# sjtuytc/betapose

Measured on AMD Instinct MI355X. Metric: frames/sec (640x480, 50-kp KPD), higher is better.
Workload: dtype f32 as an exact 3-way bf16 operand split (6 bf16 MFMA products), f32 accumulate and activations

## Files before the change

betapose_amd/_lib.py:

```python
from __future__ import annotations

import ctypes as C
import os
import threading

_HERE = os.path.dirname(os.path.abspath(__file__))
LIB_PATH = os.environ.get("BP_LIB") or os.path.join(_HERE, "libbetapose_hip.so")
_lock = threading.Lock()
_lib = None

c_float_p = C.POINTER(C.c_float)
c_double_p = C.POINTER(C.c_double)
c_int_p = C.POINTER(C.c_int)
vp = C.c_void_p

PROTOTYPES = {
    "bp_last_error": (C.c_char_p, []),
    "bp_version": (C.c_int, []),
    "bp_device_count": (C.c_int, []),
    "bp_device_name": (C.c_int, [C.c_int, C.c_char_p, C.c_int]),
    "bp_yolo_create": (C.c_int, [C.c_char_p, C.c_char_p, C.c_int, C.c_int, C.c_int, C.POINTER(vp)]),
    "bp_yolo_create_from_memory": (C.c_int, [C.c_char_p, vp, C.c_size_t, C.c_int, C.c_int, C.c_int, C.POINTER(vp)]),
    "bp_yolo_clone": (C.c_int, [vp, C.POINTER(vp)]),
    "bp_kpd_clone": (C.c_int, [vp, C.POINTER(vp)]),
    "bp_yolo_destroy": (None, [vp]),
    "bp_yolo_rows": (C.c_int, [vp]),
    "bp_yolo_attrs": (C.c_int, [vp]),
    "bp_yolo_forward": (C.c_int, [vp, vp, C.c_int, vp, vp]),
    "bp_yolo_forward_select": (C.c_int, [vp, vp, C.c_int, C.c_float, C.c_int, vp, vp, vp]),
    "bp_yolo_forward_select_classes": (C.c_int, [vp, vp, C.c_int, C.c_float, C.c_int, vp, C.c_int, vp, vp, vp]),
    "bp_yolo_select": (C.c_int, [vp, C.c_int, C.c_int, C.c_int, C.c_float, C.c_int, vp, vp]),
    "bp_yolo_tap_count": (C.c_int, [vp]),
    "bp_yolo_tap_info": (C.c_int, [vp, C.c_int, C.c_char_p, C.c_int, c_int_p, c_int_p, c_int_p]),
    "bp_yolo_tap_copy": (C.c_int, [vp, C.c_int, C.c_int, vp, vp]),
    "bp_kpd_create": (C.c_int, [vp, C.c_size_t, C.c_int, C.c_int, C.c_int, C.POINTER(vp)]),
    "bp_kpd_destroy": (None, [vp]),
    "bp_kpd_forward": (C.c_int, [vp, vp, C.c_int, vp, vp]),
    "bp_kpd_forward_argmax": (C.c_int, [vp, vp, C.c_int, vp, vp, vp]),
    "bp_kpd_launch_count": (C.c_int, [vp, C.c_int]),
    "bp_kpd_tap_count": (C.c_int, [vp]),
    "bp_kpd_tap_info": (C.c_int, [vp, C.c_int, C.c_char_p, C.c_int, c_int_p, c_int_p, c_int_p]),
    "bp_kpd_tap_copy": (C.c_int, [vp, C.c_int, C.c_int, vp, vp]),
    "bp_yolo_set_policy": (C.c_int, [vp, C.c_int, C.c_int, C.c_int, C.c_int]),
    "bp_kpd_set_policy": (C.c_int, [vp, C.c_int, C.c_int, C.c_int, C.c_int]),
    "bp_yolo_set_precision": (C.c_int, [vp, C.c_int]),
    "bp_kpd_set_precision": (C.c_int, [vp, C.c_int]),
# ... 204 lines not shown
```

betapose_amd/csrc/aux_kernels.hip:

```cpp
#include "bp_common.h"

namespace bp {

__device__ __forceinline__ void store_plane(unsigned short* planes, long long idx, long long plane_elems, int np, float v) {
    if (np == 1) {
        const _Float16 h = (_Float16)v;
        planes[idx] = __builtin_bit_cast(unsigned short, h);
    } else if (np == 3) {
        const __bf16 h1 = (__bf16)v;
        const float r1 = v - (float)h1;
        const __bf16 h2 = (__bf16)r1;
        const __bf16 h3 = (__bf16)(r1 - (float)h2);
        planes[idx] = __builtin_bit_cast(unsigned short, h1);
        planes[idx + plane_elems] = __builtin_bit_cast(unsigned short, h2);
        planes[idx + 2 * plane_elems] = __builtin_bit_cast(unsigned short, h3);
    }
}

static inline int grid_for(long long n, int block = 256, int cap = 4096) {
    BP_CHECK(n < (1ll << 31), "tensor too large for 32-bit indexing");
    long long g = (n + block - 1) / block;
    return (int)(g < 1 ? 1 : (g > cap ? cap : g));
}

// ... 300 lines not shown
            o[1] = q[0] - q[2] / 2;
            o[2] = q[1] - q[3] / 2;
            o[3] = q[0] + q[2] / 2;
            o[4] = q[1] + q[3] / 2;
            o[5] = q[4];
            o[6] = q[5];
            o[7] = 0.f;
        }
    }
}
void launch_yolo_select(const float* pred, int N, int rows, int attrs, float conf, int num_classes, float* sel,
                        hipStream_t s, int sel_ld) {
    hipLaunchKernelGGL(yolo_select_kernel, dim3(N), dim3(1024), 0, s, pred, rows, attrs, conf, num_classes, sel, sel_ld);
}

__global__ __launch_bounds__(1024) void yolo_decode_select_kernel(YoloHeads hs, int reso, int attrs, int rows, float conf, int num_classes,
                                                                   float* __restrict__ sel, int sel_ld) {
    __shared__ float sv[16];
    __shared__ int si[16];
    const int n = blockIdx.x;
    const int ncls = min(num_classes, attrs - 5);
    auto locate = [&](int row, int* a) -> const float* {
        int hi = 0;
        for (int k = 1; k < hs.n; ++k)
            if (row >= hs.h[k].row_off) hi = k;
        const YoloHead& H = hs.h[hi];
        const int g = H.g, r = row - H.row_off;
        *a = r / (g * g);
        const int cell = r - *a * g * g;
        return H.t + ((long long)n * g * g + cell) * (3 * attrs) + *a * attrs;
    };
    float best = -1.f;
    int bi = 0x7fffffff;
    for (int r = threadIdx.x; r < rows; r += blockDim.x) {
        int a;
        const float* t = locate(r, &a);
        const float obj = sigmoidf_(t[4]);
        if (!(obj > conf)) continue;
        int cls = 0;
        float cm = sigmoidf_(t[5]);
        for (int k = 1; k < ncls; ++k) {
            const float v = sigmoidf_(t[5 + k]);
            if (v > cm) { cm = v; cls = k; }
        }
        if (cls != 0) continue;
        if (obj > best || (obj == best && r < bi)) { best = obj; bi = r; }
    }
    for (int off = 32; off > 0; off >>= 1) {
        const float ov = __shfl_down(best, off, 64);
        const int oi = __shfl_down(bi, off, 64);
        if (ov > best || (ov == best && oi < bi)) { best = ov; bi = oi; }
    }
    const int w = threadIdx.x >> 6;
    if ((threadIdx.x & 63) == 0) { sv[w] = best; si[w] = bi; }
    __syncthreads();
    if (threadIdx.x == 0) {
        for (int k = 1; k < (int)(blockDim.x >> 6); ++k)
            if (sv[k] > best || (sv[k] == best && si[k] < bi)) { best = sv[k]; bi = si[k]; }
        float* o = sel + (long long)n * sel_ld;
        if (best < 0.f) {
            o[0] = __int_as_float(-1);
            for (int k = 1; k < 8; ++k) o[k] = 0.f;
        } else {
            int a, hi = 0;
            const float* t = locate(bi, &a);
            for (int k = 1; k < hs.n; ++k)
                if (bi >= hs.h[k].row_off) hi = k;
            const YoloHead& H = hs.h[hi];
            const int g = H.g, r = bi - H.row_off, cell = r - a * g * g;
            const int gy = cell / g, gx = cell - gy * g;
            const float stride = (float)(reso / g);
            const float q0 = (sigmoidf_(t[0]) + (float)gx) * stride;
            const float q1 = (sigmoidf_(t[1]) + (float)gy) * stride;
            const float q2 = (expf(t[2]) * (H.aw[a] / stride)) * stride;
            const float q3 = (expf(t[3]) * (H.ah[a] / stride)) * stride;
            o[0] = __int_as_float(bi);
            o[1] = q0 - q2 / 2;
            o[2] = q1 - q3 / 2;
            o[3] = q0 + q2 / 2;
            o[4] = q1 + q3 / 2;
            o[5] = sigmoidf_(t[4]);
            o[6] = sigmoidf_(t[5]);
            o[7] = 0.f;
        }
    }
}
void launch_yolo_decode_select(const YoloHead* heads, int nheads, int N, int reso, int attrs, int rows, float conf, int num_classes,
                               float* sel, hipStream_t s, int sel_ld) {
    BP_CHECK(nheads <= 4, "at most 4 yolo heads");
    YoloHeads hs;
    hs.n = nheads;
    for (int i = 0; i < nheads; ++i) hs.h[i] = heads[i];
    hipLaunchKernelGGL(yolo_decode_select_kernel, dim3(N), dim3(1024), 0, s, hs, reso, attrs, rows, conf, num_classes, sel, sel_ld);
}

struct PredRows {
    const float* P;
    int attrs;
    __device__ __forceinline__ const float* row(int r) const { return P + (long long)r * attrs; }
    __device__ __forceinline__ float attr(const float* q, int k) const { return q[k]; }
    __device__ __forceinline__ void box(int, const float* q, float* b) const { b[0] = q[0]; b[1] = q[1]; b[2] = q[2]; b[3] = q[3]; }
};
struct HeadRows {
    const YoloHeads* hs;
    int n, attrs, reso;
    __device__ __forceinline__ int head_of(int r) const {
        int hi = 0;
        for (int k = 1; k < hs->n; ++k)
// ... 565 lines not shown
```

betapose_amd/csrc/bp_common.h:

```cpp
#pragma once
#include <hip/hip_runtime.h>
#include <cstdint>
#include <cstdio>
#include <mutex>
#include <set>
#include <stdexcept>
#include <string>
#include <utility>

namespace bp {

struct Error : std::runtime_error {
    using std::runtime_error::runtime_error;
};

#define BP_HIP(expr)                                                                      \
    do {                                                                                  \
        hipError_t _e = (expr);                                                           \
        if (_e != hipSuccess)                                                             \
            throw ::bp::Error(std::string(#expr) + ": " + hipGetErrorString(_e) + " @" +  \
                              __FILE__ + ":" + std::to_string(__LINE__));                 \
    } while (0)

#define BP_CHECK(cond, msg)                                                               \
// ... 61 lines not shown
    int out_np;
    int skip_f32;
    const unsigned short* res16;
    int net_prec;
    int abl;
    const unsigned short* wbd;
    const unsigned short* wpl;
    float* pool_out;
    int hy_full, hy_splits, hy_cps;
    int xcd_home;
    int* xcc_of;
    int* err_word;
    int* tickets_local;
    int mtiles, n_tiles;
    int work_blocks;
    const void* pf_ptr;
    int pf_first;
    int pf_ntn, pf_splits, pf_cps, pf_nchunks;
    int pf_tile_stride, pf_chunk_bytes;
    int pf_cap;
};

enum Precision : int { PREC_F32 = 0, PREC_F16 = 1, PREC_BF16X3 = 2, PREC_F16_RES = 3 };

enum ConvTile : int { TILE_64x64 = 0, TILE_128x64 = 1, TILE_W64_1x1 = 2, TILE_W64_1x2 = 3, TILE_W64_2x1 = 5, TILE_W64_2x2 = 6,
                      TILE_KG1 = 7, TILE_KG2 = 8, TILE_KG4 = 9,
                      TILE_RD4 = 10, TILE_RD8 = 11,
                      TILE_64x64_BD = 12,
                      TILE_PL64 = 13,
                      TILE_PL128 = 14,
// ... 87 lines not shown
int avgpool_parts(int HW);
void launch_avgpool(const float* in, int in_ld, float* out, int N, int HW, int C, hipStream_t s);
void launch_fc(const float* in, const float* w, const float* bias, float* out, int N, int Cin, int Cout,
               int act, int in_parts, float in_scale, hipStream_t s);

struct YoloHead {
    const float* t;
    int g;
    float aw[3], ah[3];
    int row_off;
};
void launch_yolo_decode(const YoloHead* heads, int nheads, int N, int reso, int attrs, int rows,
                        float* pred, hipStream_t s);
void launch_yolo_select(const float* pred, int N, int rows, int attrs, float conf, int num_classes,
                        float* sel, hipStream_t s, int sel_ld = 8);
void launch_yolo_decode_select(const YoloHead* heads, int nheads, int N, int reso, int attrs, int rows, float conf, int num_classes,
                               float* sel, hipStream_t s, int sel_ld = 8);
#define BP_MAX_SCENE_CLASSES 16
struct YoloClassList {
    int n;
    int id[BP_MAX_SCENE_CLASSES];
};
YoloClassList make_class_list(const int* class_ids, int K, int num_classes, int attrs);
void launch_yolo_select_classes(const float* pred, int N, int rows, int attrs, float conf, int num_classes, const YoloClassList& cl,
                                float* sel, hipStream_t s, int ld_image, int ld_slot);
void launch_yolo_decode_select_classes(const YoloHead* heads, int nheads, int N, int reso, int attrs, int rows, float conf,
                                       int num_classes, const YoloClassList& cl, float* sel, hipStream_t s, int ld_image, int ld_slot);
#define BP_MAX_CANDIDATES 8
void launch_yolo_select_nms(const float* pred, int N, int rows, int attrs, float conf, int num_classes, int class_id, float nms_conf,
                            int C, float* sel, int* count, hipStream_t s, int ld_image, int ld_slot);
void launch_yolo_decode_select_nms(const YoloHead* heads, int nheads, int N, int reso, int attrs, int rows, float conf, int num_classes,
                                   int class_id, float nms_conf, int C, float* sel, int* count, hipStream_t s, int ld_image,
// ... 27 lines not shown
```

betapose_amd/csrc/c_api.cpp:

```cpp
#include "../../include/betapose_hip.h"

#include <algorithm>
#include <cmath>
#include <cstdlib>
#include <cstring>
#include <fstream>
#include <memory>
#include <sstream>
#include <vector>

#include "annotate.h"
#include "engine.h"
#include "frame_chain.h"
#include "frame_io.h"
#include "icp.h"
#include "pose_tail.h"
#include "raster.h"

static thread_local std::string g_err;

#define BP_TRY try {
#define BP_CATCH                                   \
    }                                              \
    catch (const std::exception& e) {              \
// ... 333 lines not shown
                                   int K, float* d_pred, float* d_sel, void* stream) {
    BP_TRY
    BP_CHECK(K >= 1 && K <= BP_MAX_SCENE_CLASSES, "class list: 1 to 16 class ids (BP_MAX_SCENE_CLASSES)");
    BP_CHECK(y && d_img && class_ids && d_sel, "null argument");
    y->net->forward_classes(d_img, false, batch, d_pred, conf, num_classes, class_ids, K, d_sel, (hipStream_t)stream);
    return 0;
    BP_CATCH
}

int bp_yolo_select(const float* d_pred, int batch, int rows, int attrs, float conf, int num_classes, float* d_sel,
                   void* stream) {
    BP_TRY
    BP_CHECK(d_pred && d_sel && batch >= 1 && rows >= 1 && attrs >= 6, "bad argument");
    bp::launch_yolo_select(d_pred, batch, rows, attrs, conf, num_classes, d_sel, (hipStream_t)stream);
    BP_HIP(hipGetLastError());
    return 0;
    BP_CATCH
}

int bp_yolo_select_nms(const float* d_pred, int batch, int rows, int attrs, float conf, int num_classes, int class_id,
                       float nms_conf, int max_candidates, float* d_sel, int* d_counts, void* stream) {
    BP_TRY
    BP_CHECK(d_pred && d_sel && d_counts && batch >= 1 && rows >= 1 && attrs >= 6, "bad argument");
    bp::launch_yolo_select_nms(d_pred, batch, rows, attrs, conf, num_classes, class_id, nms_conf, max_candidates, d_sel, d_counts,
                               (hipStream_t)stream, max_candidates * BP_SEL_FLOATS, BP_SEL_FLOATS);
    BP_HIP(hipGetLastError());
    return 0;
    BP_CATCH
}

// ... 1529 lines not shown
```

betapose_amd/csrc/conv_igemm.hip:

```cpp
#include <cstdlib>

#include "conv_dev.h"

namespace bp {

template <int TM, int TN, int VEC, class P>
__device__ __forceinline__ void conv_igemm_body(const P& p, const int bp_bid, float* const smem, int* const s_last_p) {
    constexpr int BM = 64 * TM, BN = 64 * TN;
    constexpr int RA = BM / 32, RB = BN / 32;
    float (*As)[BM * LDS_LD] = reinterpret_cast<float (*)[BM * LDS_LD]>(smem);
    float (*Bs)[BN * LDS_LD] = reinterpret_cast<float (*)[BN * LDS_LD]>(smem + 2 * BM * LDS_LD);
    constexpr int LDT = BN + 4;
    static_assert(BM * LDT <= 2 * (BM + BN) * LDS_LD, "LDS too small for the staged epilogue");

    const unsigned long long t_entry = p.stamps ? bp_clock() : 0ull;
    const int tid = threadIdx.x;
    const int lane = tid & 63;
    const int wave = tid >> 6;
    const int wm = wave >> 1, wn = wave & 1;
    const int n_tiles_n = p.CoutPad / BN;
    const int split = bp_bid % p.splits;
    const int tile_id = bp_bid / p.splits;
    const int tile_n = tile_id % n_tiles_n;
    const int tile_m = tile_id / n_tiles_n;
// ... 488 lines not shown
        __syncthreads();
    }
#define BH_STAMP(k_) if (p.stamps && tid == 0) p.stamps[(long long)(tile_id * p.splits + split) * 8 + (k_)] = bp_clock();
    if (p.stamps && tid == 0) p.stamps[(long long)(tile_id * p.splits + split) * 8 + 0] = t_entry;
    BH_STAMP(3);

    const int w_row0 = wm * (BM / 2), w_col0 = wn * (BN / 2);
    const bool kg_has_acc = KG == 1 || kgrp == 0;
#define BP_NT (256 * KG)
#define BP_SLAST (*s_last_p)
#define BP_EARLY_BIAS bias_early
#define BP_HAS_ACC kg_has_acc
#define BP_TAIL_STAMP(k_) BH_STAMP(k_)
#define BP_EP_RES_SCALE true
#define BP_EP_UP2
#include "conv_tail.inc"
#undef BP_EP_UP2
#undef BP_EP_RES_SCALE
#undef BP_HAS_ACC
#undef BP_EARLY_BIAS
#undef BP_TAIL_STAMP
#undef BP_NT
#undef BP_SLAST
    if (p.stamps) { asm volatile("s_waitcnt vmcnt(0)" ::: "memory"); BH_STAMP(4); }
#undef BH_STAMP
#undef BH_AS
#undef BH_BS
#undef BH_ADDR
#undef BH_LOAD
#undef BH_PARKED
#undef BH_LOAD_BD
// ... 405 lines not shown
            hipExtLaunchKernelGGL((conv_igemm_kernel<TM, TN, 0>), grid, dim3(256), 0, s, g_conv_prof->e0, g_conv_prof->e1, 0, p);
    } else if (vec == 1) {
        hipLaunchKernelGGL((conv_igemm_kernel<TM, TN, 1>), grid, dim3(256), 0, s, p);
    } else if (vec == 2) {
        hipLaunchKernelGGL((conv_igemm_kernel<TM, TN, 2>), grid, dim3(256), 0, s, p);
    } else {
        hipLaunchKernelGGL((conv_igemm_kernel<TM, TN, 0>), grid, dim3(256), 0, s, p);
    }
}

template <int TM, int TN, int NP, bool BD = false>
static void launch_h_t(const ConvParams& p, hipStream_t s) {
    constexpr int BM = 64 * TM, BN = 64 * TN;
    ConvParams q = p;
    conv_grid_setup(q, BM, BN);
    dim3 grid(conv_grid_blocks(q));
    if (g_conv_prof)
        hipExtLaunchKernelGGL((conv_igemm_h_kernel<TM, TN, NP, BD>), grid, dim3(256), 0, s, g_conv_prof->e0, g_conv_prof->e1, 0, q);
    else
        hipLaunchKernelGGL((conv_igemm_h_kernel<TM, TN, NP, BD>), grid, dim3(256), 0, s, q);
}

int conv_vec_mode(const ConvParams& p) {
    if ((p.Cin % 32 == 0) && (p.in_ld % 4 == 0) && p.ksize <= 8) return 1;
    if (p.cin_pack == 4 && p.Cin <= 4 && p.ksize <= 8) return 2;
    return 0;
}

bool conv_h16_eligible(const ConvParams& p) {
    return (p.w16 != nullptr || p.w16s != nullptr) && (p.Cin % 32 == 0) && (p.in_ld % 4 == 0) && p.ksize <= 8;
// ... 17 lines not shown
        launch_stem7(p, s);
    } else if (conv_tile_is_pl(tile)) {
        launch_conv_pl(p, tile, s);
    } else if (conv_tile_is_halo(tile)) {
        launch_conv_halo(p, tile, s);
    } else if (tile == TILE_64x64_BD && p.mfma_mode == PREC_BF16X3) {
        BP_CHECK(conv_h16_eligible(p) && p.w16s != nullptr, "filters-direct tile needs the stage-packed filter copy and Cin % 32 == 0");
        BP_CHECK((long long)3 * p.CoutPad * p.Kpad * 2 < (long long)OOB, "filter planes too large for 32-bit offsets");
        launch_h_t<1, 1, 3, true>(p, s);
    } else if (tile == TILE_BD_K2) {
        BP_CHECK(p.mfma_mode == PREC_BF16X3 && conv_h16_eligible(p) && p.w16s != nullptr, "filters-direct K2 tile: bf16x3 mode, stage-packed filter copy, Cin % 32 == 0");
        BP_CHECK((long long)3 * p.CoutPad * p.Kpad * 2 < (long long)OOB, "filter planes too large for 32-bit offsets");
        BP_CHECK(!p.xcd_home && !p.pf_ptr, "filters-direct K2 tile: no latency-mode layouts");
        ConvParams q = p;
        conv_grid_setup(q, 64, 64);
        if (g_conv_prof) hipExtLaunchKernelGGL(conv_igemm_bdk2_kernel, dim3(conv_grid_blocks(q)), dim3(512), 0, s, g_conv_prof->e0, g_conv_prof->e1, 0, q);
        else hipLaunchKernelGGL(conv_igemm_bdk2_kernel, dim3(conv_grid_blocks(q)), dim3(512), 0, s, q);
#ifdef BP_EXPERIMENTAL
    } else if (conv_tile_is_w64(tile)) {
        launch_conv_w64(p, tile, s);
    } else if (conv_tile_is_kg(tile)) {
        launch_conv_kg(p, tile, s);
    } else if (conv_tile_is_rd(tile)) {
        launch_conv_rd(p, tile, s);
    } else if (p.mfma_mode == PREC_F16 && conv_h16_eligible(p)) {
        switch (tile) {
            case TILE_64x64_BD:
                BP_CHECK(p.w16s != nullptr, "filters-direct tile needs the stage-packed filter copy");
                launch_h_t<1, 1, 1, true>(p, s);
                break;
// ... 20 lines not shown
```

betapose_amd/csrc/conv_tail.inc:

```
#ifdef BP_HAS_ACC
    const bool EP_HAS_ACC = BP_HAS_ACC;
#else
    constexpr bool EP_HAS_ACC = true;
#endif
    constexpr int EP_TPR = BN / 4;
    constexpr int EP_ROWS = BP_NT / EP_TPR;
    constexpr int EP_PASSES = BM / EP_ROWS;
#ifndef BP_EP_PF_MAX
#define BP_EP_PF_MAX 4
#define BP_TAIL_OWN_PF_MAX
#endif
    constexpr int EP_PF = EP_PASSES <= BP_EP_PF_MAX ? 1 : 0;
    const int ep_n4 = (tid % EP_TPR) * 4;
    const int ep_n = n0 + ep_n4;
    const int ep_row0 = tid / EP_TPR;
#ifdef BP_EARLY_BIAS
    const f32x4 ep_bias4 = BP_EARLY_BIAS;
#else
    const f32x4 ep_bias4 = *reinterpret_cast<const f32x4*>(p.bias + min(ep_n, p.CoutPad - 4));
#endif
#ifdef BP_EP_PIXSHUF
    const bool ep_ps = p.store_mode == ST_PIXSHUF && p.res == nullptr && ((p.Cout >> 2) & 3) == 0 && p.pool_out == nullptr;
#else
    constexpr bool ep_ps = false;
#endif
#ifdef BP_EP_RES_SCALE
    constexpr bool EP_RSCALE = BP_EP_RES_SCALE;
#else
    constexpr bool EP_RSCALE = false;
#endif
    const bool ep_rs = EP_RSCALE && p.res_scale != nullptr && p.res != nullptr && p.store_mode == ST_NHWC;
#ifdef BP_EP_UP2
    const bool ep_up = p.store_mode == ST_UP2 && p.res == nullptr && p.pool_out == nullptr;
#else
    constexpr bool ep_up = false;
#endif
    const bool ep_vec_ok = (p.store_mode == ST_NHWC || ep_ps || ep_up) && (p.res_scale == nullptr || ep_rs) && (p.out_ld & 3) == 0 && (p.Cout & 3) == 0 &&
                        (p.res == nullptr || (p.res_ld & 3) == 0);
    const bool ep_r16 = p.res16 != nullptr;
    const int ep_rb = ep_r16 ? 2 : 4;
    const __amdgpu_buffer_rsrc_t ep_rsrcR = __builtin_amdgcn_make_buffer_rsrc(
        ep_r16 ? (void*)const_cast<unsigned short*>(p.res16) : (void*)const_cast<float*>(p.res ? p.res : p.out), 0,
        (int)min((long long)p.M * (p.res ? p.res_ld : p.out_ld) * ep_rb, (long long)OOB), 0x00020000);
    const unsigned ep_off_r = (unsigned)(((m0 + ep_row0) * p.res_ld + ep_n) * ep_rb), ep_step_r = (unsigned)(EP_ROWS * p.res_ld * ep_rb);
    f32x4 ep_rpre[EP_PF ? EP_PASSES : 1];
#define BP_PREFETCH_RES()                                                                              \
    if (EP_PF && ep_vec_ok && p.res != nullptr && ep_n < p.Cout) {                                              \
        _Pragma("unroll") for (int pass = 0; pass < (EP_PF ? EP_PASSES : 1); ++pass)                         \
            ep_rpre[pass] = load_res4(ep_rsrcR, ep_off_r + pass * ep_step_r, ep_r16);                              \
    }
#ifndef BP_SPLITS
#define BP_SPLITS p.splits
#define BP_SLAB_TILE tile_id
// ... 94 lines not shown
                            }
                    }
                }
        };
        if (EP_HAS_ACC) {
            if (p.xcd_home) combine(std::integral_constant<int, 1>{});
            else combine(std::integral_constant<int, 16>{});
        }
        if (p.xcd_home && !xcd_home_verify(p, tile_id, &BP_SLAST)) return;
    }

    BP_TAIL_STAMP(6);
#if defined(BP_EXPERIMENTAL) && defined(BP_ABLATE_EPILOGUE)
    if (ep_vec_ok) return;
#endif
    if (ep_vec_ok) {
#ifdef BP_EP_SLABS
        constexpr int EP_SLABS = BP_EP_SLABS;
#else
        constexpr int EP_SLABS = 1;
#endif
        constexpr int SLAB_ROWS = BM / EP_SLABS;
        constexpr int SLAB_PASSES = EP_PASSES / EP_SLABS;
        static_assert(EP_SLABS == 1 || (EP_PF == 0 && SLAB_ROWS % (32 * TM) == 0 && EP_PASSES % EP_SLABS == 0), "epilogue slabs");
        const __amdgpu_buffer_rsrc_t rsrcO =
            __builtin_amdgcn_make_buffer_rsrc(p.out, 0, (int)min((long long)p.M * p.out_ld * ((ep_ps || ep_up) ? 16 : 4), (long long)OOB), 0x00020000);
        const int mode = p.act * 3 + (p.res ? (p.res_after_act ? 2 : 1) : 0);
        const PlaneDesc ep_pd = make_plane_desc(p);
#pragma unroll
        for (int sl = 0; sl < EP_SLABS; ++sl) {
            if (sl > 0) __syncthreads();
            if (EP_HAS_ACC && (EP_SLABS == 1 || w_row0 / SLAB_ROWS == sl)) {
#pragma unroll
                for (int i = 0; i < TM; ++i)
#pragma unroll
                    for (int j = 0; j < TN; ++j)
#pragma unroll
                        for (int r = 0; r < 16; ++r) {
                            const int row = w_row0 - sl * SLAB_ROWS + i * 32 + (r & 3) + 8 * (r >> 2) + 4 * (lane >> 5);
                            smem[row * LDT + w_col0 + j * 32 + (lane & 31)] = acc[i][j][r];
                        }
            }
            __syncthreads();
            if constexpr (EP_SLABS == 1 && BM == 64) {
                if (p.pool_out != nullptr && tid < BN && n0 + tid < p.Cout) {
                    const int nvalid = min(BM, p.M - m0);
                    float s = 0.f;
                    for (int r = 0; r < nvalid; ++r) s += smem[r * LDT + tid];
                    p.pool_out[(long long)(m0 / BM) * p.Cout + n0 + tid] = s + (float)nvalid * p.bias[n0 + tid];
                }
            }
            if (ep_n < p.Cout) {
                const float* srow = &smem[ep_row0 * LDT + ep_n4];
                const unsigned off_o = (unsigned)(((m0 + sl * SLAB_ROWS + ep_row0) * p.out_ld + ep_n) * 4), step_o = (unsigned)(EP_ROWS * p.out_ld * 4);
                const unsigned off_r = ep_off_r + (unsigned)(sl * SLAB_ROWS * p.res_ld * ep_rb);
                PixShufRows ep_rows;
                if (ep_ps) {
                    const int cq = p.Cout >> 2, ij = ep_n / cq, cc = ep_n - ij * cq;
                    ep_rows.m_first = m0 + sl * SLAB_ROWS + ep_row0; ep_rows.m_step = EP_ROWS; ep_rows.M = p.M;
                    ep_rows.hw = p.OH * p.OW; ep_rows.OW = p.OW; ep_rows.OH = p.OH; ep_rows.out_ld = p.out_ld;
                    ep_rows.sub = (unsigned)((((ij >> 1) * (2 * p.OW) + (ij & 1)) * p.out_ld + cc) * 4);
                    ep_rows.rcp_hw = 1.0f / (float)ep_rows.hw; ep_rows.rcp_ow = 1.0f / (float)p.OW;
                }
                Up2Rows ep_uprows;
                if (ep_up) {
                    ep_uprows.m_first = m0 + sl * SLAB_ROWS + ep_row0; ep_uprows.m_step = EP_ROWS; ep_uprows.M = p.M;
// ... 44 lines not shown
```

betapose_amd/csrc/engine.cpp:

```cpp
#include "engine.h"

#include <algorithm>
#include <cmath>
#include <cstdlib>
#include <cstring>
#include <sstream>

namespace bp {

Arena::~Arena() {
    for (void* p : ptrs_) (void)hipFree(p);
}
void* Arena::alloc_bytes(size_t bytes) {
    void* p = nullptr;
    bytes = (bytes + 255) & ~size_t(255);
    BP_HIP(hipMalloc(&p, bytes));
    ptrs_.push_back(p);
    total_ += bytes;
    return p;
}
float* Arena::alloc(size_t n) { return static_cast<float*>(alloc_bytes(n * sizeof(float))); }

Tensor Net::new_tensor(int H, int W, int C) {
    Tensor t;
// ... 866 lines not shown
            YoloHead h{};
            h.t = t.p; h.g = t.H; h.row_off = row_off;
            for (int a = 0; a < 3; ++a) {
                BP_CHECK(mask[a] >= 0 && 2 * mask[a] + 1 < (int)an.size(), "anchor mask");
                h.aw[a] = (float)an[2 * mask[a]];
                h.ah[a] = (float)an[2 * mask[a] + 1];
            }
            heads_.push_back(h);
            f32_readers_.push_back(t.p);
            row_off += 3 * t.H * t.W;
        }
    }
    BP_CHECK(!heads_.empty() && heads_.size() <= 4, "cfg must have 1..4 yolo layers");
    rows_ = row_off;
    pred_ = arena_.alloc((size_t)max_batch * rows_ * attrs_);
    finalize();
}

void YoloNet::run_net(const float* d_img, bool nhwc_input, int batch, hipStream_t s) {
    BP_CHECK(batch >= 1 && batch <= max_batch_, "batch out of range");
    if (nhwc_input) {
        if (d_img != in_nhwc_)
            BP_HIP(hipMemcpyAsync(in_nhwc_, d_img, (size_t)batch * reso_ * reso_ * 3 * sizeof(float),
                                  hipMemcpyDeviceToDevice, s));
    } else {
        launch_nchw_to_nhwc(d_img, in_nhwc_, batch, 3, reso_, reso_, s);
    }
    run_ops(batch, s);
}

void YoloNet::forward(const float* d_img, bool nhwc_input, int batch, float* d_pred, float conf, int num_classes,
                      float* d_sel, hipStream_t s, int sel_ld) {
    run_net(d_img, nhwc_input, batch, s);
    static const bool two_kernels = std::getenv("BP_NO_DECODE_FUSION") != nullptr;
    if (d_sel && !d_pred && !two_kernels) {
        launch_yolo_decode_select(heads_.data(), (int)heads_.size(), batch, reso_, attrs_, rows_, conf, num_classes, d_sel, s, sel_ld);
    } else {
        float* pred = d_pred ? d_pred : pred_;
        launch_yolo_decode(heads_.data(), (int)heads_.size(), batch, reso_, attrs_, rows_, pred, s);
        if (d_sel) launch_yolo_select(pred, batch, rows_, attrs_, conf, num_classes, d_sel, s, sel_ld);
    }
    BP_HIP(hipGetLastError());
}

void YoloNet::forward_classes(const float* d_img, bool nhwc_input, int batch, float* d_pred, float conf, int num_classes,
                              const int* class_ids, int K, float* d_sel, hipStream_t s, int ld_image, int ld_slot) {
    const YoloClassList cl = make_class_list(class_ids, K, num_classes, attrs_);
    BP_CHECK(d_sel, "null select buffer");
    if (ld_image <= 0) ld_image = K * ld_slot;
    run_net(d_img, nhwc_input, batch, s);
    if (!d_pred) {
// ... 199 lines not shown
```

betapose_amd/csrc/engine.h:

```cpp
#pragma once
#include <map>
#include <memory>
#include <mutex>
#include <string>
#include <vector>

#include "bp_common.h"
#include "conv_plan.h"

namespace bp {

struct Tensor {
    float* p = nullptr;
    int H = 0, W = 0, C = 0;
    int ld = 0;
};

class Arena {
public:
    ~Arena();
    float* alloc(size_t n_floats);
    void* alloc_bytes(size_t bytes);
    size_t total_bytes() const { return total_; }
private:
// ... 135 lines not shown
    void forward(const float* d_img, bool nhwc_input, int batch, float* d_pred, float conf, int num_classes,
                 float* d_sel, hipStream_t s, int sel_ld = 8);
    void forward_classes(const float* d_img, bool nhwc_input, int batch, float* d_pred, float conf, int num_classes,
                         const int* class_ids, int K, float* d_sel, hipStream_t s, int ld_image = 0, int ld_slot = 8);
    void forward_nms(const float* d_img, bool nhwc_input, int batch, float* d_pred, float conf, int num_classes, int class_id,
                     float nms_conf, int C, float* d_sel, int* d_count, hipStream_t s, int ld_image = 0, int ld_slot = 8);
    float* input_nhwc() { return in_nhwc_; }
    float* pred_buffer() { return pred_; }
private:
    void run_net(const float* d_img, bool nhwc_input, int batch, hipStream_t s);
    std::string cfg_text_;
    size_t n_floats_ = 0;
    int reso_, rows_ = 0, attrs_ = 0;
    float* in_nhwc_ = nullptr;
    float* pred_ = nullptr;
    std::vector<YoloHead> heads_;
};

class KpdNet : public Net {
public:
    KpdNet(const float* stream, size_t n_floats, int n_classes, int max_batch, int inH = 320, int inW = 256,
           std::shared_ptr<WeightStore> store = nullptr);
    KpdNet* clone() const { return new KpdNet(nullptr, n_floats_, n_classes_, max_batch_, inH_, inW_, store_); }
    int out_c() const { return outC_; }
    int out_h() const { return inH_ / 4; }
    int out_w() const { return inW_ / 4; }
    int in_h() const { return inH_; }
    int in_w() const { return inW_; }
    void forward(const float* d_inps, bool nhwc_input, int batch, float* d_hm, float* d_kp, hipStream_t s, int kp_ld = 0);
    float* input_nhwc() { return in_nhwc_; }
// ... 17 lines not shown
```

betapose_amd/ops.py:

```python
from __future__ import annotations

import ctypes as C
from typing import Optional

import numpy as np

from . import _lib

ACT = {"linear": 0, "leaky": 1, "relu": 2}
STORE = {"nhwc": 0, "up2": 1, "pixshuf": 2, "nchw": 3}
_F16, _B3 = 256, 512
TILE = {"auto": -1, "64x64": 0, "128x64": 1, "stem3": 20, "stem7": 28, "64x64_f16": _F16, "128x64_f16": _F16 + 1, "64x64_b3": _B3, "bd_b3": _B3 + 12,
        "bd_f16": _F16 + 12, "halo64_b3": _B3 + 21, "halo128_b3": _B3 + 22, "halo64k2_b3": _B3 + 23, "bdk2_b3": _B3 + 24}
for _n, _i in (("w1x1", 2), ("w1x2", 3), ("w2x1", 5), ("w2x2", 6), ("pl64", 13), ("pl128", 14), ("pl128x64", 15), ("pl256x128", 16), ("pl128s", 17), ("pl64k2", 18), ("pl64bd", 19), ("plh128", 25), ("s1", 26), ("p3", 27)):
    TILE[_n + "_f16"] = _F16 + _i
    TILE[_n + "_b3"] = _B3 + _i
for _n, _i in (("kg1", 7), ("kg2", 8), ("kg4", 9), ("rd4", 10), ("rd8", 11)):
    TILE[_n + "_b3"] = _B3 + _i


def conv2d_nhwc(x, weight, bias=None, stride: int = 1, pad: int = 0, act: str = "linear", store: str = "nhwc",
                res=None, res_after_act: bool = False, tile: str = "auto", splits: int = 0, iters: int = 0,
                planes: bool = False, out=None):
    import torch
# ... 20 lines not shown
        raise ValueError("out must be a contiguous float32 tensor of shape %s on %s" % (shape, x.device))
    ms = C.c_float(0)
    pl = None
    if planes:
        assert store != "nchw", "NCHW outputs (the heat-maps) have no operand planes"
        pl = torch.zeros((1 if TILE[tile] < _B3 else 3,) + tuple(out.shape), device=x.device, dtype=torch.int16)
    _lib.check(_lib.lib().bp_conv2d_planes(x.data_ptr(), N, H, W, Cin, w.ctypes.data, b.ctypes.data if b is not None else None,
                                           Cout, k, stride, pad, ACT[act], STORE[store],
                                           res.contiguous().data_ptr() if res is not None else None, int(res_after_act),
                                           TILE[tile], int(splits), out.data_ptr(), pl.data_ptr() if planes else None,
                                           int(iters), C.byref(ms), _lib.current_stream()))
    ret = (out,) + ((pl,) if planes else ()) + ((ms.value,) if iters > 0 else ())
    return ret if len(ret) > 1 else out


def crop(frames_bgr_u8, sel=None, boxes=None, reso: int = 416, oh: int = 320, ow: int = 256, nchw: bool = True):
    import torch
    _lib.require_gpu()
    f = frames_bgr_u8.contiguous()
    B, H, W, _ = f.shape
    out = torch.empty((B, 3, oh, ow) if nchw else (B, oh, ow, 3), device=f.device, dtype=torch.float32)
    pts = torch.empty((B, 8), device=f.device, dtype=torch.float32)
    _lib.check(_lib.lib().bp_crop(f.data_ptr(), B, H, W, sel.contiguous().data_ptr() if sel is not None else None, reso,
                                  boxes.contiguous().data_ptr() if boxes is not None else None,
                                  out.data_ptr() if nchw else None, None if nchw else out.data_ptr(), pts.data_ptr(),
                                  oh, ow, _lib.current_stream()))
    return out, pts


def crop_candidates(frames_bgr_u8, candidates: int, sel=None, boxes=None, reso: int = 416, oh: int = 320, ow: int = 256,
# ... 223 lines not shown
```

include/betapose_hip.h:

```cpp
#ifndef BETAPOSE_HIP_H
#define BETAPOSE_HIP_H

#include <stddef.h>
#include <stdint.h>

#ifdef __cplusplus
extern "C" {
#endif

typedef struct bp_yolo bp_yolo;
typedef struct bp_kpd bp_kpd;
typedef struct bp_pipeline bp_pipeline;
typedef struct bp_scene bp_scene;
typedef struct bp_cands bp_cands;

#define BP_RESULT_FLOATS 316
#define BP_KP_FLOATS 6
#define BP_SEL_FLOATS 8
#define BP_MAX_SCENE_CLASSES 16
#define BP_MAX_CANDIDATES 8
#define BP_MERGED_FLOATS 152

#define BP_POSE_DOUBLES 166
#define BP_PNP_MAX_POINTS 64
// ... 5 lines not shown

int bp_yolo_create(const char* cfg_path, const char* weights_path, int reso, int max_batch, int device, bp_yolo** out);
int bp_yolo_create_from_memory(const char* cfg_text, const float* stream, size_t n_floats, int reso, int max_batch,
                               int device, bp_yolo** out);
int bp_yolo_clone(const bp_yolo* y, bp_yolo** out);
void bp_yolo_destroy(bp_yolo* y);
int bp_yolo_rows(const bp_yolo* y);
int bp_yolo_attrs(const bp_yolo* y);
int bp_yolo_forward(bp_yolo* y, const float* d_img_nchw, int batch, float* d_pred, void* stream);
int bp_yolo_forward_select(bp_yolo* y, const float* d_img_nchw, int batch, float conf, int num_classes, float* d_pred,
                           float* d_sel, void* stream);
int bp_yolo_forward_select_classes(bp_yolo* y, const float* d_img_nchw, int batch, float conf, int num_classes,
                                   const int* class_ids, int K, float* d_pred, float* d_sel, void* stream);
int bp_yolo_select(const float* d_pred, int batch, int rows, int attrs, float conf, int num_classes, float* d_sel,
                   void* stream);
int bp_yolo_select_nms(const float* d_pred, int batch, int rows, int attrs, float conf, int num_classes, int class_id,
                       float nms_conf, int max_candidates, float* d_sel, int* d_counts, void* stream);
int bp_yolo_forward_select_nms(bp_yolo* y, const float* d_img_nchw, int batch, float conf, int num_classes, int class_id,
                               float nms_conf, int max_candidates, float* d_pred, float* d_sel, int* d_counts, void* stream);
int bp_yolo_tap_count(const bp_yolo* y);
int bp_yolo_tap_info(const bp_yolo* y, int i, char* name, int cap, int* C, int* H, int* W);
int bp_yolo_tap_copy(bp_yolo* y, int i, int batch, float* d_out_nchw, void* stream);

int bp_kpd_create(const float* stream, size_t n_floats, int n_classes, int max_batch, int device, bp_kpd** out);
int bp_kpd_clone(const bp_kpd* k, bp_kpd** out);
void bp_kpd_destroy(bp_kpd* k);
int bp_kpd_forward(bp_kpd* k, const float* d_inps_nchw, int batch, float* d_hm, void* stream);
int bp_kpd_forward_argmax(bp_kpd* k, const float* d_inps_nchw, int batch, float* d_hm, float* d_kp, void* stream);
int bp_kpd_launch_count(bp_kpd* k, int batch);
int bp_kpd_tap_count(const bp_kpd* k);
// ... 220 lines not shown
```

Baseline: 1010.

## Split YOLO decode-select across blocks and add wide vectorized conv epilogue stores

The fused YOLO decode+select kernel now spreads each image's rows over up to 64 blocks of 256 threads. A last-block-done ticket in a persistent workspace combines the per-block best candidates, so one 1024-thread block per image no longer serializes the scan. Separately, the 3-plane bf16 conv epilogue gains a wide-store path for NHWC and NCHW outputs that do not qualify for the existing vector path. That path stages bias in LDS and issues 128-bit buffer stores. It also adds a test API entry point and an env switch to disable the wide stores, and the ticket workspace relies on correct atomic ordering.

```diff
diff --git a/betapose_amd/_lib.py b/betapose_amd/_lib.py
--- a/betapose_amd/_lib.py
+++ b/betapose_amd/_lib.py
@@ -30,6 +30,7 @@
     "bp_yolo_forward_select": (C.c_int, [vp, vp, C.c_int, C.c_float, C.c_int, vp, vp, vp]),
     "bp_yolo_forward_select_classes": (C.c_int, [vp, vp, C.c_int, C.c_float, C.c_int, vp, C.c_int, vp, vp, vp]),
     "bp_yolo_select": (C.c_int, [vp, C.c_int, C.c_int, C.c_int, C.c_float, C.c_int, vp, vp]),
+    "bp_yolo_decode_select_heads": (C.c_int, [vp, vp, vp, C.c_int, C.c_int, C.c_int, C.c_int, C.c_float, C.c_int, C.c_int, vp, vp]),
     "bp_yolo_tap_count": (C.c_int, [vp]),
     "bp_yolo_tap_info": (C.c_int, [vp, C.c_int, C.c_char_p, C.c_int, c_int_p, c_int_p, c_int_p]),
     "bp_yolo_tap_copy": (C.c_int, [vp, C.c_int, C.c_int, vp, vp]),
diff --git a/betapose_amd/csrc/aux_kernels.hip b/betapose_amd/csrc/aux_kernels.hip
--- a/betapose_amd/csrc/aux_kernels.hip
+++ b/betapose_amd/csrc/aux_kernels.hip
@@ -338,11 +338,15 @@
     hipLaunchKernelGGL(yolo_select_kernel, dim3(N), dim3(1024), 0, s, pred, rows, attrs, conf, num_classes, sel, sel_ld);
 }
 
-__global__ __launch_bounds__(1024) void yolo_decode_select_kernel(YoloHeads hs, int reso, int attrs, int rows, float conf, int num_classes,
-                                                                   float* __restrict__ sel, int sel_ld) {
-    __shared__ float sv[16];
-    __shared__ int si[16];
-    const int n = blockIdx.x;
+static constexpr int DS_THREADS = 256, DS_MAX_BLOCKS = 64;
+struct DsPair { float best; int row; };
+struct DsImage { int ticket, pad; DsPair pairs[DS_MAX_BLOCKS]; };
+__global__ __launch_bounds__(DS_THREADS) void yolo_decode_select_kernel(YoloHeads hs, int reso, int attrs, int rows, float conf, int num_classes,
+                                                                         float* __restrict__ sel, int sel_ld, DsImage* ws) {
+    __shared__ float sv[DS_THREADS / 64];
+    __shared__ int si[DS_THREADS / 64];
+    __shared__ int s_last;
+    const int n = blockIdx.y;
     const int ncls = min(num_classes, attrs - 5);
     auto locate = [&](int row, int* a) -> const float* {
         int hi = 0;
@@ -356,7 +360,7 @@
     };
     float best = -1.f;
     int bi = 0x7fffffff;
-    for (int r = threadIdx.x; r < rows; r += blockDim.x) {
+    for (int r = blockIdx.x * DS_THREADS + threadIdx.x; r < rows; r += gridDim.x * DS_THREADS) {
         int a;
         const float* t = locate(r, &a);
         const float obj = sigmoidf_(t[4]);
@@ -378,9 +382,26 @@
     const int w = threadIdx.x >> 6;
     if ((threadIdx.x & 63) == 0) { sv[w] = best; si[w] = bi; }
     __syncthreads();
-    if (threadIdx.x == 0) {
-        for (int k = 1; k < (int)(blockDim.x >> 6); ++k)
-            if (sv[k] > best || (sv[k] == best && si[k] < bi)) { best = sv[k]; bi = si[k]; }
+    if (threadIdx.x != 0) return;
+    for (int k = 1; k < DS_THREADS / 64; ++k)
+        if (sv[k] > best || (sv[k] == best && si[k] < bi)) { best = sv[k]; bi = si[k]; }
+    if (gridDim.x > 1) {
+        DsPair* const pairs = ws[n].pairs;
+        __hip_atomic_store(&pairs[blockIdx.x].best, best, __ATOMIC_RELAXED, __HIP_MEMORY_SCOPE_AGENT);
+        __hip_atomic_store(&pairs[blockIdx.x].row, bi, __ATOMIC_RELAXED, __HIP_MEMORY_SCOPE_AGENT);
+        const int ticket = __hip_atomic_fetch_add(&ws[n].ticket, 1, __ATOMIC_ACQ_REL, __HIP_MEMORY_SCOPE_AGENT);
+        if (ticket != (int)gridDim.x - 1) return;
+        __hip_atomic_store(&ws[n].ticket, 0, __ATOMIC_RELAXED, __HIP_MEMORY_SCOPE_AGENT);
+        best = -1.f;
+        bi = 0x7fffffff;
+        for (int k = 0; k < (int)gridDim.x; ++k) {
+            const float ov = __hip_atomic_load(&pairs[k].best, __ATOMIC_RELAXED, __HIP_MEMORY_SCOPE_AGENT);
+            const int oi = __hip_atomic_load(&pairs[k].row, __ATOMIC_RELAXED, __HIP_MEMORY_SCOPE_AGENT);
+            if (ov > best || (ov == best && oi < bi)) { best = ov; bi = oi; }
+        }
+    }
+    {
+#pragma clang fp contract(off)
         float* o = sel + (long long)n * sel_ld;
         if (best < 0.f) {
             o[0] = __int_as_float(-1);
@@ -409,13 +430,17 @@
         }
     }
 }
+size_t yolo_decode_select_ws_bytes(int N) { return (size_t)N * sizeof(DsImage); }
 void launch_yolo_decode_select(const YoloHead* heads, int nheads, int N, int reso, int attrs, int rows, float conf, int num_classes,
-                               float* sel, hipStream_t s, int sel_ld) {
+                               float* sel, hipStream_t s, int sel_ld, void* ws) {
     BP_CHECK(nheads <= 4, "at most 4 yolo heads");
     YoloHeads hs;
     hs.n = nheads;
     for (int i = 0; i < nheads; ++i) hs.h[i] = heads[i];
-    hipLaunchKernelGGL(yolo_decode_select_kernel, dim3(N), dim3(1024), 0, s, hs, reso, attrs, rows, conf, num_classes, sel, sel_ld);
+    const int want = (rows + DS_THREADS - 1) / DS_THREADS;
+    const int blocks = !ws || want < 1 ? 1 : want > DS_MAX_BLOCKS ? DS_MAX_BLOCKS : want;
+    hipLaunchKernelGGL(yolo_decode_select_kernel, dim3(blocks, N), dim3(DS_THREADS), 0, s, hs, reso, attrs, rows, conf, num_classes, sel, sel_ld,
+                       static_cast<DsImage*>(ws));
 }
 
 struct PredRows {
diff --git a/betapose_amd/csrc/bp_common.h b/betapose_amd/csrc/bp_common.h
--- a/betapose_amd/csrc/bp_common.h
+++ b/betapose_amd/csrc/bp_common.h
@@ -99,6 +99,7 @@
     int* tickets_local;
     int mtiles, n_tiles;
     int work_blocks;
+    int ep_elementwise;
     const void* pf_ptr;
     int pf_first;
     int pf_ntn, pf_splits, pf_cps, pf_nchunks;
@@ -216,8 +217,9 @@
                         float* pred, hipStream_t s);
 void launch_yolo_select(const float* pred, int N, int rows, int attrs, float conf, int num_classes,
                         float* sel, hipStream_t s, int sel_ld = 8);
+size_t yolo_decode_select_ws_bytes(int N);
 void launch_yolo_decode_select(const YoloHead* heads, int nheads, int N, int reso, int attrs, int rows, float conf, int num_classes,
-                               float* sel, hipStream_t s, int sel_ld = 8);
+                               float* sel, hipStream_t s, int sel_ld = 8, void* ws = nullptr);
 #define BP_MAX_SCENE_CLASSES 16
 struct YoloClassList {
     int n;
diff --git a/betapose_amd/csrc/c_api.cpp b/betapose_amd/csrc/c_api.cpp
--- a/betapose_amd/csrc/c_api.cpp
+++ b/betapose_amd/csrc/c_api.cpp
@@ -371,6 +371,39 @@
     BP_CHECK(d_pred && d_sel && batch >= 1 && rows >= 1 && attrs >= 6, "bad argument");
     bp::launch_yolo_select(d_pred, batch, rows, attrs, conf, num_classes, d_sel, (hipStream_t)stream);
     BP_HIP(hipGetLastError());
+    return 0;
+    BP_CATCH
+}
+
+int bp_yolo_decode_select_heads(const float* const* d_heads, const int* grids, const float* anchors, int nheads, int batch, int reso,
+                                int attrs, float conf, int num_classes, int fused, float* d_sel, void* stream) {
+    BP_TRY
+    BP_CHECK(d_heads && grids && anchors && d_sel && nheads >= 1 && nheads <= 4 && batch >= 1 && attrs >= 6, "bad argument");
+    hipStream_t s = (hipStream_t)stream;
+    bp::YoloHead h[4];
+    int rows = 0;
+    for (int i = 0; i < nheads; ++i) {
+        BP_CHECK(d_heads[i] && grids[i] >= 1 && reso >= grids[i], "bad head");
+        h[i].t = d_heads[i]; h[i].g = grids[i]; h[i].row_off = rows;
+        for (int a = 0; a < 3; ++a) { h[i].aw[a] = anchors[(i * 3 + a) * 2]; h[i].ah[a] = anchors[(i * 3 + a) * 2 + 1]; }
+        rows += 3 * grids[i] * grids[i];
+    }
+    void* tmp = nullptr;
+    if (fused) {
+        const size_t bytes = bp::yolo_decode_select_ws_bytes(batch);
+        BP_HIP(hipMalloc(&tmp, bytes));
+        BP_HIP(hipMemsetAsync(tmp, 0, bytes, s));
+        for (int rep = 0; rep < 2; ++rep) bp::launch_yolo_decode_select(h, nheads, batch, reso, attrs, rows, conf, num_classes, d_sel, s, 8, tmp);
+    } else {
+        BP_HIP(hipMalloc(&tmp, (size_t)batch * rows * attrs * sizeof(float)));
+        bp::launch_yolo_decode(h, nheads, batch, reso, attrs, rows, (float*)tmp, s);
+        bp::launch_yolo_select((const float*)tmp, batch, rows, attrs, conf, num_classes, d_sel, s);
+    }
+    const hipError_t e = hipGetLastError();
+    const hipError_t e2 = hipStreamSynchronize(s);
+    (void)hipFree(tmp);
+    BP_HIP(e);
+    BP_HIP(e2);
     return 0;
     BP_CATCH
 }
diff --git a/betapose_amd/csrc/conv_igemm.hip b/betapose_amd/csrc/conv_igemm.hip
--- a/betapose_amd/csrc/conv_igemm.hip
+++ b/betapose_amd/csrc/conv_igemm.hip
@@ -526,7 +526,10 @@
 #define BP_TAIL_STAMP(k_) BH_STAMP(k_)
 #define BP_EP_RES_SCALE true
 #define BP_EP_UP2
+#define BP_EP_WIDE (BD && NP == 3)
+    static_assert(!(BD && NP == 3) || IgemmHLds<TM, TN, NP, BD>::FLOATS >= BM * LDT + BN, "wide stores: the tile's biases sit behind the staging tile");
 #include "conv_tail.inc"
+#undef BP_EP_WIDE
 #undef BP_EP_UP2
 #undef BP_EP_RES_SCALE
 #undef BP_HAS_ACC
@@ -962,6 +965,7 @@
     constexpr int BM = 64 * TM, BN = 64 * TN;
     ConvParams q = p;
     conv_grid_setup(q, BM, BN);
+    q.ep_elementwise = std::getenv("BP_NO_WIDE_STORES") != nullptr;
     dim3 grid(conv_grid_blocks(q));
     if (g_conv_prof)
         hipExtLaunchKernelGGL((conv_igemm_h_kernel<TM, TN, NP, BD>), grid, dim3(256), 0, s, g_conv_prof->e0, g_conv_prof->e1, 0, q);
@@ -1009,6 +1013,7 @@
         BP_CHECK(!p.xcd_home && !p.pf_ptr, "filters-direct K2 tile: no latency-mode layouts");
         ConvParams q = p;
         conv_grid_setup(q, 64, 64);
+        q.ep_elementwise = std::getenv("BP_NO_WIDE_STORES") != nullptr;
         if (g_conv_prof) hipExtLaunchKernelGGL(conv_igemm_bdk2_kernel, dim3(conv_grid_blocks(q)), dim3(512), 0, s, g_conv_prof->e0, g_conv_prof->e1, 0, q);
         else hipLaunchKernelGGL(conv_igemm_bdk2_kernel, dim3(conv_grid_blocks(q)), dim3(512), 0, s, q);
 #ifdef BP_EXPERIMENTAL
diff --git a/betapose_amd/csrc/conv_tail.inc b/betapose_amd/csrc/conv_tail.inc
--- a/betapose_amd/csrc/conv_tail.inc
+++ b/betapose_amd/csrc/conv_tail.inc
@@ -37,6 +37,19 @@
 #endif
     const bool ep_vec_ok = (p.store_mode == ST_NHWC || ep_ps || ep_up) && (p.res_scale == nullptr || ep_rs) && (p.out_ld & 3) == 0 && (p.Cout & 3) == 0 &&
                         (p.res == nullptr || (p.res_ld & 3) == 0);
+#ifdef BP_EP_WIDE
+    constexpr bool EP_WIDE = BP_EP_WIDE;
+#else
+    constexpr bool EP_WIDE = false;
+#endif
+    int ep_wide = 0;
+    if constexpr (EP_WIDE) {
+        static_assert(BM == 64 && BN == 64, "wide stores: 64x64 tile");
+        const bool plain = !p.ep_elementwise && p.res == nullptr && p.res_scale == nullptr && p.pool_out == nullptr && p.out16 == nullptr &&
+                           (reinterpret_cast<unsigned long long>(p.out) & 15ull) == 0ull;
+        if (plain && !ep_vec_ok && p.store_mode == ST_NHWC && p.out_ld == p.Cout && p.CoutPad == BN) ep_wide = 1;
+        if (plain && p.store_mode == ST_NCHW && ((p.OH * p.OW) & 63) == 0 && (long long)p.M * p.Cout * 4 < (long long)OOB) ep_wide = 2;
+    }
     const bool ep_r16 = p.res16 != nullptr;
     const int ep_rb = ep_r16 ? 2 : 4;
     const __amdgpu_buffer_rsrc_t ep_rsrcR = __builtin_amdgcn_make_buffer_rsrc(
@@ -161,7 +174,7 @@
 #if defined(BP_EXPERIMENTAL) && defined(BP_ABLATE_EPILOGUE)
     if (ep_vec_ok) return;
 #endif
-    if (ep_vec_ok) {
+    if (ep_vec_ok || (EP_WIDE && ep_wide != 0)) {
 #ifdef BP_EP_SLABS
         constexpr int EP_SLABS = BP_EP_SLABS;
 #else
@@ -170,8 +183,9 @@
         constexpr int SLAB_ROWS = BM / EP_SLABS;
         constexpr int SLAB_PASSES = EP_PASSES / EP_SLABS;
         static_assert(EP_SLABS == 1 || (EP_PF == 0 && SLAB_ROWS % (32 * TM) == 0 && EP_PASSES % EP_SLABS == 0), "epilogue slabs");
+        static_assert(!EP_WIDE || EP_SLABS == 1, "wide stores: one staging slab");
         const __amdgpu_buffer_rsrc_t rsrcO =
-            __builtin_amdgcn_make_buffer_rsrc(p.out, 0, (int)min((long long)p.M * p.out_ld * ((ep_ps || ep_up) ? 16 : 4), (long long)OOB), 0x00020000);
+            __builtin_amdgcn_make_buffer_rsrc(p.out, 0, (int)min((long long)p.M * ((EP_WIDE && ep_wide != 0) ? p.Cout : p.out_ld) * ((ep_ps || ep_up) ? 16 : 4), (long long)OOB), 0x00020000);
         const int mode = p.act * 3 + (p.res ? (p.res_after_act ? 2 : 1) : 0);
         const PlaneDesc ep_pd = make_plane_desc(p);
 #pragma unroll
@@ -188,6 +202,7 @@
                             smem[row * LDT + w_col0 + j * 32 + (lane & 31)] = acc[i][j][r];
                         }
             }
+            if (EP_WIDE && ep_wide != 0 && tid < EP_TPR) *reinterpret_cast<f32x4*>(smem + BM * LDT + ep_n4) = ep_bias4;
             __syncthreads();
             if constexpr (EP_SLABS == 1 && BM == 64) {
                 if (p.pool_out != nullptr && tid < BN && n0 + tid < p.Cout) {
@@ -197,6 +212,42 @@
                     p.pool_out[(long long)(m0 / BM) * p.Cout + n0 + tid] = s + (float)nvalid * p.bias[n0 + tid];
                 }
             }
+            if (EP_WIDE && ep_wide == 1) {
+                const float* const sbias = smem + BM * LDT;
+                const int total = min(BM, p.M - m0) * p.Cout;
+                const float rcp_c = 1.0f / (float)p.Cout;
+                for (int e0 = tid * 4; e0 < total; e0 += BP_NT * 4) {
+                    int row = fast_div(e0, p.Cout, rcp_c), col = e0 - row * p.Cout;
+                    float v[4];
+#pragma unroll
+                    for (int k = 0; k < 4; ++k) {
+                        v[k] = apply_act(smem[row * LDT + col] + sbias[col], p.act);
+                        if (++col == p.Cout) { col = 0; ++row; }
+                    }
+                    const int off = (m0 * p.Cout + e0) * 4;
+                    if (e0 + 4 <= total) {
+                        __builtin_amdgcn_raw_buffer_store_b128(u32x4{__float_as_uint(v[0]), __float_as_uint(v[1]), __float_as_uint(v[2]), __float_as_uint(v[3])}, rsrcO, off, 0, 0);
+                    } else {
+#pragma unroll
+                        for (int k = 0; k < 3; ++k)
+                            if (e0 + k < total) __builtin_amdgcn_raw_buffer_store_b32(__float_as_uint(v[k]), rsrcO, off + 4 * k, 0, 0);
+                    }
+                }
+            } else if (EP_WIDE && ep_wide == 2) {
+                const float* const sbias = smem + BM * LDT;
+                const int hw = p.OH * p.OW;
+                const int b = m0 / hw, pix0 = m0 - b * hw;
+                const int nch = min(BN, p.Cout - n0);
+                for (int f = tid; f < nch * 16; f += BP_NT) {
+                    const int c = f >> 4, j4 = (f & 15) * 4;
+                    const float bias = sbias[c];
+                    float v[4];
+#pragma unroll
+                    for (int k = 0; k < 4; ++k) v[k] = apply_act(smem[(j4 + k) * LDT + c] + bias, p.act);
+                    const int off = (((b * p.Cout + n0 + c) * hw) + pix0 + j4) * 4;
+                    __builtin_amdgcn_raw_buffer_store_b128(u32x4{__float_as_uint(v[0]), __float_as_uint(v[1]), __float_as_uint(v[2]), __float_as_uint(v[3])}, rsrcO, off, 0, 0);
+                }
+            } else
             if (ep_n < p.Cout) {
                 const float* srow = &smem[ep_row0 * LDT + ep_n4];
                 const unsigned off_o = (unsigned)(((m0 + sl * SLAB_ROWS + ep_row0) * p.out_ld + ep_n) * 4), step_o = (unsigned)(EP_ROWS * p.out_ld * 4);
diff --git a/betapose_amd/csrc/engine.cpp b/betapose_amd/csrc/engine.cpp
--- a/betapose_amd/csrc/engine.cpp
+++ b/betapose_amd/csrc/engine.cpp
@@ -904,6 +904,8 @@
     BP_CHECK(!heads_.empty() && heads_.size() <= 4, "cfg must have 1..4 yolo layers");
     rows_ = row_off;
     pred_ = arena_.alloc((size_t)max_batch * rows_ * attrs_);
+    select_ws_ = arena_.alloc_bytes(yolo_decode_select_ws_bytes(max_batch));
+    BP_HIP(hipMemset(select_ws_, 0, yolo_decode_select_ws_bytes(max_batch)));
     finalize();
 }
 
@@ -924,7 +926,7 @@
     run_net(d_img, nhwc_input, batch, s);
     static const bool two_kernels = std::getenv("BP_NO_DECODE_FUSION") != nullptr;
     if (d_sel && !d_pred && !two_kernels) {
-        launch_yolo_decode_select(heads_.data(), (int)heads_.size(), batch, reso_, attrs_, rows_, conf, num_classes, d_sel, s, sel_ld);
+        launch_yolo_decode_select(heads_.data(), (int)heads_.size(), batch, reso_, attrs_, rows_, conf, num_classes, d_sel, s, sel_ld, select_ws_);
     } else {
         float* pred = d_pred ? d_pred : pred_;
         launch_yolo_decode(heads_.data(), (int)heads_.size(), batch, reso_, attrs_, rows_, pred, s);
diff --git a/betapose_amd/csrc/engine.h b/betapose_amd/csrc/engine.h
--- a/betapose_amd/csrc/engine.h
+++ b/betapose_amd/csrc/engine.h
@@ -173,6 +173,7 @@
     int reso_, rows_ = 0, attrs_ = 0;
     float* in_nhwc_ = nullptr;
     float* pred_ = nullptr;
+    void* select_ws_ = nullptr;
     std::vector<YoloHead> heads_;
 };
 
diff --git a/betapose_amd/ops.py b/betapose_amd/ops.py
--- a/betapose_amd/ops.py
+++ b/betapose_amd/ops.py
@@ -58,6 +58,21 @@
     return ret if len(ret) > 1 else out
 
 
+def yolo_decode_select(heads, anchors, reso: int, confidence: float, num_classes: int = 80, fused: bool = True):
+    import torch
+    _lib.require_gpu()
+    heads = [h.contiguous() for h in heads]
+    B, attrs = heads[0].shape[0], heads[0].shape[3] // 3
+    assert all(h.dtype == torch.float32 and h.shape[0] == B and h.shape[1] == h.shape[2] and h.shape[3] == 3 * attrs for h in heads)
+    ptrs = (C.c_void_p * len(heads))(*[h.data_ptr() for h in heads])
+    grids = (C.c_int * len(heads))(*[h.shape[1] for h in heads])
+    an = np.ascontiguousarray(anchors, dtype=np.float32).reshape(len(heads), 3, 2)
+    sel = torch.empty((B, 8), device=heads[0].device, dtype=torch.float32)
+    _lib.check(_lib.lib().bp_yolo_decode_select_heads(ptrs, grids, an.ctypes.data, len(heads), B, int(reso), attrs, float(confidence),
+                                                      int(num_classes), int(fused), sel.data_ptr(), _lib.current_stream()))
+    return sel
+
+
 def crop(frames_bgr_u8, sel=None, boxes=None, reso: int = 416, oh: int = 320, ow: int = 256, nchw: bool = True):
     import torch
     _lib.require_gpu()
diff --git a/include/betapose_hip.h b/include/betapose_hip.h
--- a/include/betapose_hip.h
+++ b/include/betapose_hip.h
@@ -43,6 +43,8 @@
                                    const int* class_ids, int K, float* d_pred, float* d_sel, void* stream);
 int bp_yolo_select(const float* d_pred, int batch, int rows, int attrs, float conf, int num_classes, float* d_sel,
                    void* stream);
+int bp_yolo_decode_select_heads(const float* const* d_heads, const int* grids, const float* anchors, int nheads, int batch, int reso,
+                                int attrs, float conf, int num_classes, int fused, float* d_sel, void* stream);
 int bp_yolo_select_nms(const float* d_pred, int batch, int rows, int attrs, float conf, int num_classes, int class_id,
                        float nms_conf, int max_candidates, float* d_sel, int* d_counts, void* stream);
 int bp_yolo_forward_select_nms(bp_yolo* y, const float* d_img_nchw, int batch, float conf, int num_classes, int class_id,
```

Result: no change. 1007 (-0.3%).
